# AbrahamSanders/realtime-codec-agent

Measured on AMD Instinct MI355X. Metric: batch-encode audio-hours/hour (+ xRT and p50 frame-step latency of 1 duplex stream in `duplex`), higher is better.
Workload: dtype f32; 1 GPU; batch MagiCodec-style encode, 16 kHz stereo, 0.1 s chunks / 2.0 s context, 256 windows per step (BASELINE configs[1]); codebook=131072x16

## Files before the change

include/rca.h:

```cpp
#ifndef RCA_H
#define RCA_H

#include <stdint.h>

#ifdef __cplusplus
extern "C" {
#endif

#define RCA_OK 0
#define RCA_ERR_ARG -1
#define RCA_ERR_HIP -2
#define RCA_ERR_STATE -3
#define RCA_ERR_MISSING -4

#define RCA_MAX_STAGES 8

typedef struct rca_codec rca_codec_t;
typedef struct rca_lm rca_lm_t;

#define RCA_F32 0
#define RCA_BF16 1
#define RCA_Q8_0 2
#define RCA_F16 3
#define RCA_Q6_K 5
// ... 44 lines not shown
                                     int64_t chunk_begin, int64_t chunk_end, int64_t* codes_dev,
                                     int64_t codes_per_channel, void* stream);

int rca_codec_encode_rows_dev(rca_codec_t* h, const float* audio_dev, const int64_t* src_off_dev, int32_t B, int32_t T, int32_t n_keep,
                              int64_t* codes_dev, const int64_t* dst_off_dev, int64_t span, void* stream);

int rca_codec_encode_tail_dev(rca_codec_t* h, const float* pcm_dev, int32_t B, int32_t T, int32_t n_keep,
                              int64_t* codes_dev, void* stream);
int rca_codec_decode_tail_dev(rca_codec_t* h, const int64_t* codes_dev, int32_t B, int32_t F, int32_t n_samples,
                              float* pcm_dev, void* stream);
int rca_codec_encode_tail(rca_codec_t* h, const float* pcm_host, int32_t B, int32_t T, int32_t n_keep, int64_t* codes_host);
int rca_codec_decode_tail(rca_codec_t* h, const int64_t* codes_host, int32_t B, int32_t F, int32_t n_samples, float* pcm_host);
int rca_codec_set_stream_graphs(rca_codec_t* h, int32_t enable);
int rca_codec_set_mfma_mode(rca_codec_t* h, int32_t mode);
int rca_codec_receptive_field(const rca_codec_t* h, int32_t* enc_left_frames, int32_t* dec_left_frames);
int rca_codec_set_window_trim(rca_codec_t* h, int32_t enable);

int rca_codec_decode(rca_codec_t* h, const int64_t* codes_host, int32_t B, int32_t F, float* pcm_host);
int rca_codec_decode_dev(rca_codec_t* h, const int64_t* codes_dev, int32_t B, int32_t F, float* pcm_dev,
                         void* stream);

int rca_codec_encoder_dev(rca_codec_t* h, const float* pcm_dev, int32_t B, int32_t T, float* ze_dev, void* stream);
int rca_codec_quantize_dev(rca_codec_t* h, const float* ze_dev, int64_t rows, int64_t* codes_dev, void* stream);
int rca_codec_decoder_dev(rca_codec_t* h, const float* zq_dev, int32_t B, int32_t F, float* pcm_dev, void* stream);
int rca_codec_codebook_dev(rca_codec_t* h, const float** out_dev);

int rca_codec_codebook(rca_codec_t* h, float* out_host);

int rca_codec_encode_tap(rca_codec_t* h, const float* pcm_host, int32_t B, int32_t T, int32_t layer,
                         float* out_host, int64_t out_numel);

int rca_codec_encode_tap_bf16(rca_codec_t* h, const float* pcm_host, int32_t B, int32_t T, int32_t layer,
                              uint16_t* hi_host, uint16_t* lo_host, int64_t numel);

int rca_codec_set_variant(rca_codec_t* h, int32_t variant);

int rca_codec_profile(rca_codec_t* h, int32_t enable);
int rca_codec_profile_read(rca_codec_t* h, int32_t kclass, double* total_ms, int64_t* launches, double* flops,
                           double* bytes);

typedef struct {
    int32_t vocab_size;
    int32_t hidden;
    int32_t n_layers;
    int32_t n_heads;
    int32_t n_kv_heads;
    int32_t head_dim;
    int32_t ffn;
    int32_t n_ctx;
    float rms_eps;
    float rope_theta;
    int32_t rope_scaling;
    float rope_factor;
    float rope_low_freq_factor;
    float rope_high_freq_factor;
    int32_t rope_orig_ctx;
    int32_t logits_all;
    int32_t decode_weights;
} rca_lm_config_t;

typedef struct {
    int32_t top_k;
    float top_p;
    float min_p;
    float temp;
    uint32_t seed;
// ... 78 lines not shown
```

realtime_codec_agent_amd/_native.py:

```python
from __future__ import annotations

import ctypes as C
import os
import subprocess
from typing import Dict, Iterable, List, Optional, Tuple

import numpy as np

_PKG_DIR = os.path.dirname(os.path.abspath(__file__))
CSRC_DIR = os.path.join(_PKG_DIR, "csrc")
LIB_PATH = os.environ.get("RCA_LIB_PATH") or os.path.join(_PKG_DIR, "librca_hip.so")
HIP_SOURCES = ["rca_codec.hip", "rca_lm.hip"]
HIPCC_FLAGS = ["--offload-arch=gfx950", "-O3", "-ffp-contract=off", "-std=c++17", "-fPIC", "-shared",
               "-Wno-unused-result", "-mllvm", "-amdgpu-kernarg-preload-count=14"]

MAX_STAGES = 8
RCA_F32, RCA_BF16, RCA_Q8_0, RCA_F16, RCA_Q4_K, RCA_Q6_K = 0, 1, 2, 3, 4, 5


class RcaError(RuntimeError):
    pass


class Q8Blocks:
# ... 215 lines not shown
                    print(" ".join(cmd))
                jobs.append((subprocess.Popen(cmd), cmd, obj))
        tmps = [obj + sfx for _, _, obj in jobs] + [LIB_PATH + sfx]
        try:
            failed = [cmd for p, cmd, _ in jobs if p.wait() != 0]
            if failed:
                raise subprocess.CalledProcessError(1, failed[0])
            for _, _, obj in jobs:
                os.replace(obj + sfx, obj)
            cmd = [hipcc, "--offload-arch=gfx950", "-shared", "-fPIC"] + objs + ["-o", LIB_PATH + sfx]
            if verbose:
                print(" ".join(cmd))
            subprocess.check_call(cmd)
            os.replace(LIB_PATH + sfx, LIB_PATH)
            with open(_stamp_path() + sfx, "w") as f:
                f.write(key + "\n")
            os.replace(_stamp_path() + sfx, _stamp_path())
        finally:
            for t in tmps + [_stamp_path() + sfx]:
                if os.path.exists(t):
                    os.remove(t)
    return LIB_PATH


_lib = None

ABI_SYMBOLS = [
    "rca_last_error", "rca_device_count", "rca_device_sync", "rca_version",
    "rca_codec_create", "rca_codec_destroy", "rca_codec_hop", "rca_codec_num_frames",
    "rca_codec_encode", "rca_codec_encode_dev", "rca_codec_encode_windows_dev", "rca_codec_encode_chunk_range_dev", "rca_codec_encode_rows_dev",
    "rca_codec_decode", "rca_codec_decode_dev",
    "rca_codec_encode_tail_dev", "rca_codec_decode_tail_dev", "rca_codec_encode_tail", "rca_codec_decode_tail", "rca_codec_set_stream_graphs", "rca_codec_receptive_field", "rca_codec_set_window_trim",
    "rca_codec_encoder_dev", "rca_codec_quantize_dev", "rca_codec_decoder_dev", "rca_codec_codebook_dev",
    "rca_codec_codebook", "rca_codec_encode_tap", "rca_codec_encode_tap_bf16", "rca_codec_set_variant", "rca_codec_sync",
    "rca_codec_profile", "rca_codec_profile_read",
    "rca_lm_create", "rca_lm_create_random", "rca_lm_destroy", "rca_lm_reset", "rca_lm_eval",
    "rca_lm_get_n_tokens", "rca_lm_set_n_tokens", "rca_lm_get_logits", "rca_lm_get_logits_row",
    "rca_lm_logits_dev", "rca_lm_sampler_init", "rca_lm_sample", "rca_lm_step", "rca_lm_token_probs",
    "rca_lm_sync", "rca_lm_set_graphs", "rca_lm_mask_head_rows", "rca_lm_set_mfma_prefill", "rca_lm_set_logits_all",
    "rca_lm_persist_codec_embeddings", "rca_lm_create_shared", "rca_lm_eval_async", "rca_lm_copy_kv", "rca_lm_swap_kv",
    "rca_lm_set_low_priority", "rca_lm_frame", "rca_lm_weight_format", "rca_lm_set_attn_fuse",
    "rca_duplex_frame", "rca_codec_workspace_sig", "rca_codec_stream_handoff", "rca_codec_codebook_size", "rca_codec_set_mfma_mode", "rca_lm_step_probe", "rca_duplex_prepare", "rca_duplex_precapture",
]


def lib():
    global _lib
    if _lib is not None:
        return _lib
    if not os.path.exists(LIB_PATH):
        raise RcaError(
            f"{LIB_PATH} not found: build the HIP extension first (python -c 'import __graft_entry__ as g; g.build()'). "
            "There is no CPU fallback for the product path."
        )
    import torch
    try:
        _lib = C.CDLL(LIB_PATH)
    except OSError as e:
        raise RcaError(f"cannot load {LIB_PATH}: {e}") from e
    _lib.rca_last_error.restype = C.c_char_p
    _lib.rca_version.restype = C.c_char_p
    return _lib


def check(rc: int, what: str = "") -> None:
    if rc != 0:
        msg = lib().rca_last_error()
# ... 40 lines not shown
```

realtime_codec_agent_amd/codec.py:

```python
from __future__ import annotations

import ctypes as C
from typing import Dict, Optional, Tuple

import numpy as np

from . import _native as N
from .codec_model import CodecConfig, init_codec_weights


class HipCodec:
    def __init__(self, cfg: CodecConfig, weights: Dict[str, np.ndarray], device: int = 0):
        self.cfg = cfg
        self.device = device
        self._lib = N.lib()
        self._h = C.c_void_p()
        tensors, keep = N.make_tensors(weights)
        ccfg = N.codec_config_c(cfg)
        N.check(self._lib.rca_codec_create(C.byref(ccfg), tensors, len(weights), device, C.byref(self._h)), "rca_codec_create")
        del keep
        self.hop = cfg.hop
        self.mfma_mode = 0

    def close(self):
# ... 59 lines not shown
    def set_mfma_mode(self, mode: int) -> None:
        N.check(self._lib.rca_codec_set_mfma_mode(self._h, int(mode)), "rca_codec_set_mfma_mode")
        self.mfma_mode = int(mode)

    def set_stream_graphs(self, enable: bool) -> None:
        N.check(self._lib.rca_codec_set_stream_graphs(self._h, int(bool(enable))), "rca_codec_set_stream_graphs")

    def codebook(self) -> np.ndarray:
        out = np.empty((self.cfg.codebook_size, self.cfg.codebook_dim), np.float32)
        N.check(self._lib.rca_codec_codebook(self._h, C.c_void_p(out.ctypes.data)), "rca_codec_codebook")
        return out

    def encode_tap(self, pcm: np.ndarray, layer: int) -> np.ndarray:
        pcm = np.ascontiguousarray(pcm, dtype=np.float32)
        B, T = pcm.shape
        F = self.num_frames(T)
        n = self.cfg.n_stages
        L = F * self.hop
        if layer == 0:
            shape = (B, self.cfg.channels[0], L)
        elif layer <= n:
            for i in range(layer):
                L //= self.cfg.strides[i]
            shape = (B, self.cfg.channels[layer], L)
        elif layer == n + 1:
            shape = (B, self.cfg.latent_dim, F)
        else:
            shape = (B * F, self.cfg.codebook_dim)
        out = np.empty(shape, np.float32)
        N.check(self._lib.rca_codec_encode_tap(self._h, C.c_void_p(pcm.ctypes.data), B, T, layer, C.c_void_p(out.ctypes.data),
                                               C.c_int64(out.size)), "rca_codec_encode_tap")
        return out

    def encode_tap_bf16(self, pcm: np.ndarray, layer: int) -> Tuple[np.ndarray, Optional[np.ndarray]]:
        pcm = np.ascontiguousarray(pcm, dtype=np.float32)
        B, T = pcm.shape
        L = self.num_frames(T) * self.hop
        for i in range(layer):
            L //= self.cfg.strides[i]
        Cn = self.cfg.channels[layer] if 0 <= layer <= self.cfg.n_stages else 0
        hi = np.empty((B, Cn // 16, L, 16), np.uint16)
        lo = np.empty_like(hi) if self.mfma_mode == 3 else None
        N.check(self._lib.rca_codec_encode_tap_bf16(self._h, C.c_void_p(pcm.ctypes.data), B, T, layer, C.c_void_p(hi.ctypes.data),
                                                    C.c_void_p(lo.ctypes.data if lo is not None else None), C.c_int64(B * Cn * L)),
                "rca_codec_encode_tap_bf16")
        unblock = lambda a: np.ascontiguousarray(a.transpose(0, 1, 3, 2).reshape(B, Cn, L))
        return unblock(hi), (unblock(lo) if lo is not None else None)

    def encode_dev(self, pcm_ptr: int, B: int, T: int, codes_ptr: int, stream: int = 0) -> None:
        N.check(self._lib.rca_codec_encode_dev(self._h, C.c_void_p(pcm_ptr), B, T, C.c_void_p(codes_ptr), C.c_void_p(stream)), "rca_codec_encode_dev")

    def decode_dev(self, codes_ptr: int, B: int, F: int, pcm_ptr: int, stream: int = 0) -> None:
        N.check(self._lib.rca_codec_decode_dev(self._h, C.c_void_p(codes_ptr), B, F, C.c_void_p(pcm_ptr), C.c_void_p(stream)), "rca_codec_decode_dev")

    def encode_tail_dev(self, pcm_ptr: int, B: int, T: int, n_keep: int, codes_ptr: int, stream: int = 0) -> None:
        N.check(self._lib.rca_codec_encode_tail_dev(self._h, C.c_void_p(pcm_ptr), B, T, n_keep, C.c_void_p(codes_ptr), C.c_void_p(stream)),
                "rca_codec_encode_tail_dev")

    def decode_tail_dev(self, codes_ptr: int, B: int, F: int, n_samples: int, pcm_ptr: int, stream: int = 0) -> None:
        N.check(self._lib.rca_codec_decode_tail_dev(self._h, C.c_void_p(codes_ptr), B, F, n_samples, C.c_void_p(pcm_ptr), C.c_void_p(stream)),
                "rca_codec_decode_tail_dev")

    def receptive_field(self) -> Tuple[int, int]:
        a, b = C.c_int32(), C.c_int32()
        N.check(self._lib.rca_codec_receptive_field(self._h, C.byref(a), C.byref(b)), "rca_codec_receptive_field")
        return a.value, b.value
# ... 199 lines not shown
```

realtime_codec_agent_amd/csrc/rca_codec.hip:

```cpp
#include <stdarg.h>

#include <algorithm>
#include <array>
#include <cmath>
#include <map>
#include <type_traits>

#include "rca_common.h"

namespace rca {
thread_local char g_err[512] = {0};
}
using namespace rca;

typedef float f32x16 __attribute__((ext_vector_type(16)));

#define RCA_LAT_MAX_FRAMES 64
#define RCA_LDS_BUDGET (152 * 1024)

typedef float f32x4 __attribute__((ext_vector_type(4)));

struct RowSrc {
    const float* base;
    int C;
// ... 683 lines not shown
                    char* const yr = reinterpret_cast<char*>(yw + (long)cu * orow);
                    *reinterpret_cast<float*>(yr + voff) = acc[wm][wn][r];
                }
        } else {
#pragma unroll
            for (int wm = 0; wm < WM; ++wm)
#pragma unroll
                for (int r = 0; r < 16; ++r) {
                    const int cu = wm * 32 + (r & 3) + 8 * (r >> 2);
                    char* const yr = reinterpret_cast<char*>(yw + (long)cu * orow);
                    if (co0 + cu + 4 * half < Cout) *reinterpret_cast<float*>(yr + voff) = acc[wm][wn][r];
                }
        }
    }
#ifdef RCA_CONV_TIMELINE
    if (tl_buf && lane == 0) {
        const long tl3 = (long)wall_clock64();
        const unsigned hw = __builtin_amdgcn_s_getreg((31 << 11) | (0 << 6) | 4);
        const unsigned xcc = __builtin_amdgcn_s_getreg((3 << 11) | (0 << 6) | 20);
        constexpr int region = KS == 4 ? 0 : KS == 8 ? 1 : KS == 10 ? 2 : KS == 16 ? 3 : KS == 3 ? 4 : 5;
        long* o = tl_buf + ((long)region * 65536 + ((blockIdx.x * RCA_CONV_WPB + wave) & 0xFFFF)) * 8;
        o[6] = tl_load | (tl_mfma << 32);
        o[7] = tl_write | ((long)nchunks << 32);
        o[0] = tl0; o[1] = tl1; o[2] = tl2; o[3] = tl3;
        o[4] = (long)hw | ((long)xcc << 32);
        o[5] = (long)KS | ((long)S << 8) | ((long)WM << 16) | ((long)wave << 24) | ((long)blockIdx.x << 32);
    }
#endif
}

template <int NWN, bool PRE>
__global__ __launch_bounds__(64, 2) void conv_first_mfma_kernel(const float* __restrict__ wp, const float* __restrict__ bias,
                                                               float* __restrict__ y, int Cout, int Lout, long Ncols, int post, float slope,
                                                               FuseIn fin) {
    constexpr int NW = NWN * 32;
    constexpr int E = (NW + 2) * 2;
    constexpr int NBLK = 2 * NWN + 1;
    constexpr int RS = 136;
    constexpr int ZERO = 128;
    constexpr int CIN = 32, KQ = CIN / 2;
    extern __shared__ __attribute__((aligned(16))) float ring[];
#ifdef RCA_CONV_TIMELINE
    long* const tl_buf = rca_prof_buf;
#endif
    RCA_TL_STAMP(tl0);
    const int lane = threadIdx.x & 63;
    const int half = lane >> 5, jl = lane & 31;
    const int n_co = Cout / 64;
    const long wg = blockIdx.x;
    const int xcd = (int)(wg & 7);
    const long seq = wg >> 3;
    const int co_tile = __builtin_amdgcn_readfirstlane((int)(seq % n_co));
    const long n0 = ((seq / n_co) * 8 + xcd) * NW;
    const int co0 = co_tile * 64;
    if (n0 >= Ncols) return;
    const long n_base = n0 > 0 ? n0 - 1 : 0;
    const int b_base = __builtin_amdgcn_readfirstlane((int)((unsigned)n_base / (unsigned)Lout));
    const int t_base = (int)(n_base - (long)b_base * Lout);
    const int lead = n0 > 0 ? 0 : 1;
    const long left = Ncols - n_base;
    const int ncol_left = left > NW + 2 ? NW + 2 : (int)left;
    auto rel_bt = [&](int dn, int& bb, int& tt) {
        int dt = dn + t_base;
        bb = dt >= Lout ? 1 : 0;
        tt = bb ? dt - Lout : dt;
    };

    const int ch_in = jl;
    float a_in[4];
#pragma unroll
    for (int m = 0; m < 4; ++m) a_in[m] = (2 * m + half < 7) ? fin.w_in[ch_in * 7 + 2 * m + half] : -0.0f;
    f32x16 b_in;
#pragma unroll
    for (int r = 0; r < 16; ++r) b_in[r] = fin.b_in[(r & 3) + 8 * (r >> 2) + 4 * half];
    long o0, o1;
    if (fin.src.row_off) {
        const long nrows = (Ncols + Lout - 1) / Lout;
        o0 = fin.src.row_off[b_base];
        o1 = fin.src.row_off[b_base + 1 < nrows ? b_base + 1 : b_base];
    } else {
        const int C = fin.src.C;
        const int c0 = b_base % C, w0 = b_base / C;
        const int c1 = c0 + 1 == C ? 0 : c0 + 1, w1 = c0 + 1 == C ? w0 + 1 : w0;
        o0 = (long)c0 * fin.src.chan_stride + (long)w0 * fin.src.win_stride;
        o1 = (long)c1 * fin.src.chan_stride + (long)w1 * fin.src.win_stride;
    }
    const long om = o0 < o1 ? o0 : o1;
    const rca_rsrc_t rs_pcm = rca_make_rsrc(fin.src.base + om, 0x7FFFFFFF);
    const unsigned prow0 = (unsigned)(o0 - om), prow1 = (unsigned)(o1 - om);
    constexpr unsigned OOB = 0x80000000u;
    auto pcm_load = [&](int bk, float (&pb)[4]) __attribute__((always_inline)) {
        const int e = 32 * bk + jl;
        const int dn = (e >> 1) - lead;
        const bool ok = e < E && dn >= 0 && dn < ncol_left;
        int bb, t;
        rel_bt(ok ? dn : 0, bb, t);
        const int i = 2 * t + (e & 1) - 3 + half;
        const unsigned ro = bb ? prow1 : prow0;
#pragma unroll
        for (int m = 0; m < 4; ++m) {
            const int j = i + 2 * m;
            const unsigned off = (ok && 2 * m + half < 7 && j >= 0 && j < fin.src.T) ? (ro + (unsigned)j) * 4u : OOB;
            pb[m] = rca_buffer_load_f32(rs_pcm, (int)off, 0, 0);
        }
    };
    auto cin_mfma = [&](int m, const float (&pb)[4], f32x16& d) __attribute__((always_inline)) {
        d = __builtin_amdgcn_mfma_f32_32x32x2f32(a_in[m], pb[m], m == 0 ? b_in : d, 0, 0, 0);
    };
    const int w_lane = 4 * half * RS + jl;
    auto cin_write = [&](int bk, f32x16& d, int r0, int r1) __attribute__((always_inline)) {
#pragma unroll
        for (int r = r0; r < r1; ++r) {
            float v = d[r];
            if (PRE) v = fmaxf(v, v * slope);
            ring[w_lane + ((r & 3) + 8 * (r >> 2)) * RS + ((32 * bk) & 127)] = v;
        }
    };

    if (lane < CIN) ring[lane * RS + ZERO] = 0.0f;
    float pa[4], pb[4];
    float4 a[2][KQ];
    {
        float p2[4];
        pcm_load(0, pa);
        pcm_load(1, pb);
        pcm_load(2, p2);
        __builtin_amdgcn_sched_barrier(0);
        const rca_rsrc_t rs_w = rca_make_rsrc(reinterpret_cast<const float4*>(wp) + (long)co_tile * 2 * KQ * 64, 0x7FFFFFFF);
#pragma unroll
        for (int wm = 0; wm < 2; ++wm)
#pragma unroll
            for (int q = 0; q < KQ; ++q) {
                const rca_f32x4_t v = rca_buffer_load_f32x4(rs_w, lane * 16, (wm * KQ + q) * 1024, 0);
                a[wm][q] = make_float4(v[0], v[1], v[2], v[3]);
            }
        __builtin_amdgcn_sched_barrier(0);
        f32x16 d0, d1;
#pragma unroll
        for (int m = 0; m < 4; ++m) { cin_mfma(m, pa, d0); cin_mfma(m, pb, d1); }
        cin_write(0, d0, 0, 16);
#pragma unroll
        for (int m = 0; m < 4; ++m) cin_mfma(m, p2, d0);
        cin_write(1, d1, 0, 16);
        cin_write(2, d0, 0, 16);
    }
    if (NBLK > 3) pcm_load(3, pa);
    if (NBLK > 4) pcm_load(4, pb);
    __builtin_amdgcn_wave_barrier();
    RCA_TL_STAMP(tl1);
#ifdef RCA_CONV_TIMELINE
    long tl_load = 1 << 30, tl_mfma = 0, tl_write = 0;
#endif

    const rca_rsrc_t rs_y = rca_make_rsrc(y + ((long)b_base * Cout + co0) * Lout, 0x7FFFFFFF);
    __builtin_amdgcn_s_setprio(RCA_CONV_EPRIO);
#pragma unroll
    for (int wn = 0; wn < NWN; ++wn) {
        RCA_TL_STAMP(ta);
        const int j = 32 * wn + jl;
        int bz, tz;
        rel_bt(1 - lead + j, bz, tz);
        const int ad0 = (half == 0 && tz == 0) ? ZERO : ((2 * j + 1 + half) & 127);
        const int ad1 = (half == 1 && tz == Lout - 1) ? ZERO : ((2 * j + 3 + half) & 127);
        f32x16 acc[2];
#pragma unroll
        for (int wm = 0; wm < 2; ++wm)
#pragma unroll
            for (int q = 0; q < 4; ++q) {
                const f32x4 bq = *reinterpret_cast<const f32x4*>(bias + co0 + wm * 32 + 8 * q + 4 * half);
#pragma unroll
                for (int jj = 0; jj < 4; ++jj) acc[wm][4 * q + jj] = bq[jj];
            }
        const bool more = 2 * wn + 4 < NBLK;
        f32x16 d;
        float bcur[4], bnxt[4];
        auto b_read = [&](int c, float (&bv)[4]) __attribute__((always_inline)) {
#pragma unroll
            for (int cl = 0; cl < 2; ++cl) {
                bv[2 * cl] = ring[ad0 + (2 * c + cl) * RS];
                bv[2 * cl + 1] = ring[ad1 + (2 * c + cl) * RS];
            }
        };
        b_read(0, bcur);
#pragma unroll
        for (int c = 0; c < KQ; ++c) {
            if (c + 1 < KQ) b_read(c + 1, bnxt);
#pragma unroll
            for (int kp = 0; kp < 4; ++kp) {
#pragma unroll
                for (int wm = 0; wm < 2; ++wm) {
                    const float4 q4 = a[wm][c];
                    const float av = kp == 0 ? q4.x : kp == 1 ? q4.y : kp == 2 ? q4.z : q4.w;
                    acc[wm] = __builtin_amdgcn_mfma_f32_32x32x2f32(av, bcur[kp], acc[wm], 0, 0, 0);
                }
                if (c == 0 && 2 * wn + 3 < NBLK) cin_mfma(kp, pa, d);
                if (c == 3 && more) cin_mfma(kp, pb, d);
            }
            if (c == 2 && 2 * wn + 3 < NBLK) cin_write(2 * wn + 3, d, 0, 16);
            if (more && c >= 4 && (c & 3) == 3) cin_write(2 * wn + 4, d, 4 * (c >> 2) - 4, 4 * (c >> 2));
            if (c == 1 && 2 * wn + 5 < NBLK) pcm_load(2 * wn + 5, pa);
            if (c == 4 && 2 * wn + 6 < NBLK) pcm_load(2 * wn + 6, pb);
            if (c + 1 < KQ) {
#pragma unroll
                for (int i = 0; i < 4; ++i) bcur[i] = bnxt[i];
            }
            __builtin_amdgcn_sched_barrier(0);
        }
        if (more) cin_write(2 * wn + 4, d, 12, 16);
        __builtin_amdgcn_wave_barrier();
        RCA_TL_STAMP(tb);
        const int dn = 1 - lead + j;
        int bb, t;
        rel_bt(dn, bb, t);
        const unsigned voff = dn < ncol_left ? ((unsigned)bb * (unsigned)(Cout * Lout) + (unsigned)t + (unsigned)(4 * half * Lout)) * 4u : OOB;
        if (post) {
#pragma unroll
            for (int wm = 0; wm < 2; ++wm)
#pragma unroll
                for (int r = 0; r < 16; ++r) acc[wm][r] = fmaxf(acc[wm][r], acc[wm][r] * slope);
        }
#pragma unroll
        for (int wm = 0; wm < 2; ++wm)
#pragma unroll
            for (int r = 0; r < 16; ++r) rca_buffer_store_f32(acc[wm][r], rs_y, (int)voff, (wm * 32 + (r & 3) + 8 * (r >> 2)) * Lout * 4, 0);
        RCA_TL_STAMP(tc);
        RCA_TL_MIN(tl_load, ta, tb); RCA_TL_ADD(tl_mfma, ta, tb); RCA_TL_ADD(tl_write, tb, tc);
    }
    if (RCA_CONV_EPRIO) __builtin_amdgcn_s_setprio(0);
    RCA_TL_STAMP(tl2);
#ifdef RCA_CONV_TIMELINE
    if (tl_buf && lane == 0) {
        const long tl3 = (long)wall_clock64();
        const unsigned hw = __builtin_amdgcn_s_getreg((31 << 11) | (0 << 6) | 4);
        const unsigned xcc = __builtin_amdgcn_s_getreg((3 << 11) | (0 << 6) | 20);
        long* o = tl_buf + ((long)blockIdx.x & 0xFFFF) * 8;
        o[6] = tl_load | (tl_mfma << 32);
        o[7] = tl_write | ((long)(2 * NWN) << 32);
        o[0] = tl0; o[1] = tl1; o[2] = tl2; o[3] = tl3;
        o[4] = (long)hw | ((long)xcc << 32);
        o[5] = 4L | (2L << 8) | (2L << 16) | ((long)blockIdx.x << 32);
    }
#endif
}

template <int KS, int S, int CIC, int FUSE>
__global__ __launch_bounds__(512) void conv1d_ws_kernel(const float* __restrict__ x, const float* __restrict__ wp,
                                                        const float* __restrict__ bias, float* __restrict__ y,
                                                        int Cin, int Lin, int Cout, int Lout, long Ncols, int nchunks,
                                                        int pre, float slope, FuseIn fin) {
    constexpr int WM = 2, WN = 2;
    constexpr int MT = WM * 32, NW = WN * 32;
    constexpr int U = ConvLds<S>::stride(NW);
    constexpr int KPC = CIC * KS / 2;
    constexpr int QPC = KPC / 4;
    constexpr int E = (NW + 2) * S;
    constexpr int RE = (E + 63) / 64;
    constexpr int padL = (KS - S + 1) / 2;
    constexpr int BUF = CIC * S * U + 4;
    constexpr int WBUF = WM * QPC * 64 * 4;
    static_assert(KPC % 4 == 0 && KPC <= 64, "chunk shape");

    extern __shared__ __attribute__((aligned(16))) float lds[];
    float* aw_all = lds;
    float* xs_all = lds + 2 * WBUF;

    const int lane = threadIdx.x & 63;
    const int half = lane >> 5;
    const int wave = __builtin_amdgcn_readfirstlane(threadIdx.x >> 6);
    const bool producer = wave >= 4;
    const int cw = wave & 3;
// ... 969 lines not shown
            for (int r = 0; r < 16; ++r) yr[(long)((r & 3) + 8 * (r >> 2)) * Lout] = acc[wm][wn][r];
        } else {
            const int Cbo = Cout / 16;
#pragma unroll
            for (int g = 0; g < 4; ++g) {
                float v[4];
#pragma unroll
                for (int j = 0; j < 4; ++j) {
                    const float a = acc[wm][wn][4 * g + j];
                    v[j] = act ? fmaxf(a, a * slope) : a;
                }
                const int ch = co0 + wm * 32 + 8 * g + 4 * half;
                const long o = (((long)b * Cbo + ch / 16) * Lout + t) * 16 + (ch & 15);
                const unsigned h0 = conv_pack_bf16x2(v[0], v[1]), h1 = conv_pack_bf16x2(v[2], v[3]);
                *reinterpret_cast<uint2*>(y_hi + o) = make_uint2(h0, h1);
                if (SPLIT) {
                    const unsigned l0 = conv_pack_bf16x2(v[0] - __uint_as_float(h0 << 16), v[1] - __uint_as_float(h0 & 0xffff0000u));
                    const unsigned l1 = conv_pack_bf16x2(v[2] - __uint_as_float(h1 << 16), v[3] - __uint_as_float(h1 & 0xffff0000u));
                    *reinterpret_cast<uint2*>(y_lo + o) = make_uint2(l0, l1);
                }
            }
        }
    }
}

struct Bf16Pack { conv_bf16raw* hi = nullptr; conv_bf16raw* lo = nullptr; float* w_in8 = nullptr; };

struct rca_codec {
    rca_codec_config_t cfg;
    int device = 0;
    hipStream_t stream = nullptr;
    int hop = 1;
    int variant = 1;
    int mfma_mode = 0;
    bool lat_mode = false;
    int enc_left_frames = 0, dec_left_frames = 0;
    bool window_trim = false;
    std::vector<ConvLayer> enc, dec;
    std::vector<Bf16Pack> bf16_packs;
    bool bf16_blk_split = true;
    float *q_in_w = nullptr, *q_in_b = nullptr;
    float *cb = nullptr, *hc = nullptr, *cbp = nullptr;
    DevBuf act[2], zbuf, keys, io_a, io_b, tail;
    void* pin = nullptr; size_t pin_cap = 0;
    struct StreamGraph { hipGraphExec_t exec = nullptr; int seen = 0; unsigned long long sig = 0; };
    std::map<std::array<int, 5>, StreamGraph> sgraphs;
    bool stream_graphs = true;
    int* err_flag = nullptr;
    hipStream_t last_stream = nullptr;
    bool last_stream_valid = false;
    hipEvent_t xev = nullptr;
    struct Prof { hipEvent_t a, b; int kclass; double flops, bytes; };
    bool profile = false;
    std::vector<Prof> prof;
    std::vector<Prof> prof_pool;
};

struct ProfScope {
    rca_codec* h; hipStream_t st; rca_codec::Prof p; bool on;
    ProfScope(rca_codec* h_, hipStream_t st_, int kclass, double flops, double bytes) : h(h_), st(st_), on(h_->profile) {
        if (!on) return;
        if (!h->prof_pool.empty()) { p = h->prof_pool.back(); h->prof_pool.pop_back(); }
        else { (void)hipEventCreate(&p.a); (void)hipEventCreate(&p.b); }
        p.kclass = kclass; p.flops = flops; p.bytes = bytes;
        (void)hipEventRecord(p.a, st);
    }
// ... 231 lines not shown
    if (hipMalloc((void**)&h->cb, (size_t)N * J * 4) != hipSuccess || hipMalloc((void**)&h->hc, (size_t)N * 4) != hipSuccess ||
        hipMalloc((void**)&h->cbp, (size_t)N * J * 4) != hipSuccess || hipMalloc((void**)&h->err_flag, 4) != hipSuccess) {
        free3();
        return bail(fail(RCA_ERR_HIP, "codebook alloc"));
    }
    (void)hipMemsetAsync(h->err_flag, 0, 4, h->stream);
#ifdef RCA_CONV_TIMELINE
    if (getenv("RCA_CONV_TIMELINE_OUT")) {
        long* b = nullptr;
        (void)hipMalloc((void**)&b, (size_t)(6 << 16) * 8 * 8);
        (void)hipMemset(b, 0, (size_t)(6 << 16) * 8 * 8);
        (void)hipMemcpyToSymbol(HIP_SYMBOL(rca_prof_buf), &b, 8);
    }
#endif
    codebook_proj_kernel<<<cdiv((long)N * J, 256), 256, 0, h->stream>>>(raw, pw, pb, h->cb, N, R, J);
    codebook_norm_pack_kernel<<<cdiv(N, 256), 256, 0, h->stream>>>(h->cb, h->hc, h->cbp, N, J);
    hipError_t e = hipStreamSynchronize(h->stream);
    free3();
    if (e != hipSuccess) return bail(fail(RCA_ERR_HIP, "codebook init: %s", hipGetErrorString(e)));
    *out = h;
    return RCA_OK;
}

extern "C" int rca_codec_hop(const rca_codec_t* h, int32_t* hop) {
    if (!h || !hop) return fail(RCA_ERR_ARG, "null");
    *hop = h->hop;
    return RCA_OK;
}
extern "C" int rca_codec_num_frames(const rca_codec_t* h, int32_t T, int32_t* F) {
    if (!h || !F || T < 0) return fail(RCA_ERR_ARG, "bad argument");
    *F = (T + h->hop - 1) / h->hop;
    return RCA_OK;
}
extern "C" int rca_codec_set_variant(rca_codec_t* h, int32_t v) {
    if (!h || v < 0 || v > 2) return fail(RCA_ERR_ARG, "variant must be 0, 1 or 2");
    h->variant = v;
    return RCA_OK;
}
extern "C" int rca_codec_sync(rca_codec_t* h) {
    if (!h) return fail(RCA_ERR_ARG, "null");
    RCA_HIP(hipSetDevice(h->device));
    RCA_HIP(hipStreamSynchronize(h->stream));
    return RCA_OK;
}

template <int KS, int S, int CIC, int WM, int WN, int FUSE, int TR, int BF = 0>
static void launch_conv_cfg(const ConvLayer& L, const float* wp, int nchunks, const float* x, float* y, int Lin, int Lc, long Ncols,
                            float slope, const FuseIn& fin, const TrInfo& tr, hipStream_t st, int act) {
    constexpr int NT = RCA_CONV_WPB * WN * 32, MT = WM * 32;
    constexpr int lds = RCA_CONV_WPB * 2 * (CIC * S * ConvLds<S>::stride(WN * 32) + 4) * 4;
    static_assert(lds <= 65536, "LDS budget");
    const long col_tiles = (cdiv(Ncols, NT) + 7) / 8 * 8;
    dim3 grid((unsigned)(col_tiles * cdiv(L.cout, MT) * (TR ? tr.s : 1)));
    if constexpr (!FUSE && !TR && BF == 0) {
        if (L.cin % CIC == 0 && nchunks * CIC == L.cin) {
            conv1d_mfma_kernel<KS, S, CIC, WM, WN, 0, 0, 0, 1><<<grid, 64 * RCA_CONV_WPB, lds, st>>>(x, wp, L.bp, y, L.cin, Lin, L.cout, Lc, Ncols, nchunks, act, slope, fin, tr);
            return;
        }
    }
    conv1d_mfma_kernel<KS, S, CIC, WM, WN, FUSE, TR, BF><<<grid, 64 * RCA_CONV_WPB, lds, st>>>(x, wp, L.bp, y, L.cin, Lin, L.cout, Lc, Ncols, nchunks, act, slope, fin, tr);
}

template <int KS, int S, int CIC>
static int launch_conv_mfma(const ConvLayer& L, const float* x, float* y, int B, int Lin, int Lout, float slope, hipStream_t st,
                            const FuseIn* fuse = nullptr, int act = -1, int bf = 0) {
    if (act < 0) act = L.pre;
    const long Ncols = (long)B * Lout;
    if (bf) {
        const FuseIn none_b{};
        const TrInfo notr_b{};
        const bool big = (long)cdiv(Ncols, 64) * cdiv(L.cout, 64) >= 2048;
#define RCA_BF_LAUNCH(FU, BFM) do { \
            if (big) launch_conv_cfg<KS, S, CIC, 2, 2, FU, 0, BFM>(L, L.wp, L.nchunks, x, y, Lin, Lout, Ncols, slope, FU ? *fuse : none_b, notr_b, st, act); \
            else launch_conv_cfg<KS, S, CIC, 1, 1, FU, 0, BFM>(L, L.wp, L.nchunks, x, y, Lin, Lout, Ncols, slope, FU ? *fuse : none_b, notr_b, st, act); } while (0)
        if constexpr (KS == 4 || KS == 8 || KS == 16) {
            if (fuse) { if (bf == 3) RCA_BF_LAUNCH(1, 3); else RCA_BF_LAUNCH(1, 1); RCA_LAUNCH_CHECK(); return RCA_OK; }
        }
        if (fuse) return fail(RCA_ERR_ARG, "internal: fused first layer of this shape has no bf16 instantiation");
        if (bf == 3) RCA_BF_LAUNCH(0, 3); else RCA_BF_LAUNCH(0, 1);
#undef RCA_BF_LAUNCH
        RCA_LAUNCH_CHECK();
        return RCA_OK;
    }
    const long waves_big = (long)cdiv(Ncols, 64) * cdiv(L.cout, 64);
#ifdef RCA_CONV_FORCE_MID
    constexpr long BIG_MIN = 1L << 40, MID_MIN = 2048;
#else
    constexpr long BIG_MIN = 8192, MID_MIN = 2048;
#endif
    const FuseIn none{};
    const TrInfo notr{};
    if (fuse) {
        static const bool wide = []() { const char* e = getenv("RCA_FUSE_WIDE"); return !(e && e[0] == '0'); }();
        if constexpr (KS == 4 && S == 2) {
            const char* mi = getenv("RCA_FUSE_MFMA_IN");
            constexpr int NWN = 4;
            if (!(mi && mi[0] == '0') && wide && waves_big >= BIG_MIN && Lout >= NWN * 32 + 3 && L.cin == 32 && L.cout % 64 == 0) {
                const long col_tiles = (cdiv(Ncols, NWN * 32) + 7) / 8 * 8;
                const dim3 grid((unsigned)(col_tiles * (L.cout / 64)));
                constexpr int lds = 32 * 136 * 4;
                if (act & 1) conv_first_mfma_kernel<NWN, true><<<grid, 64, lds, st>>>(L.wp, L.bp, y, L.cout, Lout, Ncols, act & 2, slope, *fuse);
                else conv_first_mfma_kernel<NWN, false><<<grid, 64, lds, st>>>(L.wp, L.bp, y, L.cout, Lout, Ncols, act & 2, slope, *fuse);
                RCA_LAUNCH_CHECK();
                return RCA_OK;
            }
            if (wide && waves_big >= BIG_MIN && Lout >= 131 && L.cin % 2 == 0) {
                launch_conv_cfg<4, 2, 2, 2, 4, 1, 0>(L, L.wp, L.cin / 2, x, y, Lin, Lout, Ncols, slope, *fuse, notr, st, act);
                RCA_LAUNCH_CHECK();
                return RCA_OK;
            }
        }
        if (waves_big >= BIG_MIN) launch_conv_cfg<KS, S, CIC, 2, 2, 1, 0>(L, L.wp, L.nchunks, x, y, Lin, Lout, Ncols, slope, *fuse, notr, st, act);
        else launch_conv_cfg<KS, S, CIC, 1, 1, 1, 0>(L, L.wp, L.nchunks, x, y, Lin, Lout, Ncols, slope, *fuse, notr, st, act);
    } else {
        if (waves_big >= BIG_MIN) launch_conv_cfg<KS, S, CIC, 2, 2, 0, 0>(L, L.wp, L.nchunks, x, y, Lin, Lout, Ncols, slope, none, notr, st, act);
        else if (waves_big >= MID_MIN) launch_conv_cfg<KS, S, CIC, 1, 2, 0, 0>(L, L.wp, L.nchunks, x, y, Lin, Lout, Ncols, slope, none, notr, st, act);
        else if (KS == 3 && L.cout >= 64 && waves_big >= 1024) launch_conv_cfg<KS, S, CIC, (KS == 3 ? 2 : 1), 1, 0, 0>(L, L.wp, L.nchunks, x, y, Lin, Lout, Ncols, slope, none, notr, st, act);
        else launch_conv_cfg<KS, S, CIC, 1, 1, 0, 0>(L, L.wp, L.nchunks, x, y, Lin, Lout, Ncols, slope, none, notr, st, act);
    }
    RCA_LAUNCH_CHECK();
    return RCA_OK;
}

static int launch_convtr_mfma(const ConvLayer& L, const float* x, float* y, int B, int Lin, float slope, hipStream_t st) {
    const int Lc = Lin + 1;
    const long Ncols = (long)B * Lc;
    const FuseIn none{};
    const TrInfo tr{L.s, (L.k - L.s + 1) / 2, Lin * L.s, L.cout_pad / 32};
    const long waves_big = (long)cdiv(Ncols, 64) * cdiv(L.cout, 64) * L.s;
    if (L.cout > 32 && waves_big >= 2048) launch_conv_cfg<2, 1, 16, 2, 2, 0, 1>(L, L.wp_tr, L.nchunks_tr, x, y, Lin, Lc, Ncols, slope, none, tr, st, L.pre);
    else launch_conv_cfg<2, 1, 16, 1, 1, 0, 1>(L, L.wp_tr, L.nchunks_tr, x, y, Lin, Lc, Ncols, slope, none, tr, st, L.pre);
    RCA_LAUNCH_CHECK();
    return RCA_OK;
}

template <int KS, int S, int CIC, int FUSE>
// ... 276 lines not shown
        max_elems = std::max(max_elems, (size_t)B * c.latent_dim * L);
    }
    int rc;
    if ((rc = h->act[0].ensure(max_elems * 4)) != RCA_OK) return rc;
    if ((rc = h->act[1].ensure(max_elems * 4)) != RCA_OK) return rc;
    if (bf16_blk_ok(h, tap_layer) && (double)B * max_elems < 4.0e18 && Tp / h->enc[1].s >= 64) {
        *F_out = F;
        return run_encoder_bf16(h, src, B, Tp, max_elems, st, ze_out, tap_layer, tap_dev, bf16_tap, bf16_planes);
    }
    if (bf16_tap >= 0) return fail(RCA_ERR_ARG, "bf16 tap: encode() does not take the blocked bf16 pipeline here (mfma mode %d, B=%d T=%d)", h->mfma_mode, B, src.T);
    int cur = 0;
    int L = Tp;
    size_t first = 1;
    const ConvLayer& E0 = h->enc[0];
    const ConvLayer& E1 = h->enc[1];
    const bool fuse01 = !h->lat_mode && h->variant >= 1 && tap_layer != 0 && E0.k == 7 && E1.wp && E1.k == 2 * E1.s && (double)B * E1.cin * L < 4.0e9 &&
                        ((E1.k == 4 && E1.s == 2) || (E1.k == 8 && E1.s == 4) || (E1.k == 16 && E1.s == 8)) && L / E1.s >= 67 &&
                        (double)E1.cout * (L / E1.s) < 2.6e8 &&
                        (src.row_off ? (double)src.span : (double)src.C * (double)std::labs(src.chan_stride) + (double)std::labs(src.win_stride) + src.T) < 5.0e8;
    bool prev_post = false;
    auto handoff = [&](size_t next, int Lnext) {
        return tap_layer < 0 && h->variant == 1 && !h->lat_mode && next < h->enc.size() && h->enc[next].pre && mfma_conv_ok(h, h->enc[next], B, Lnext, 0);
    };
    if (fuse01) {
        float* y = h->act[cur].as<float>();
        FuseIn fin{src, E0.w, E0.b};
        const float slope = c.leaky_slope;
        const int Lout = L / E1.s;
        {
            ProfScope ps(h, st, 0, 2.0 * E1.cin * E1.k * E1.cout * (double)B * Lout + 2.0 * E0.k * E0.cout * (double)B * L,
                         4.0 * ((double)B * src.T + (double)B * E1.cout * Lout + (double)E1.cin * E1.k * E1.cout));
            prev_post = handoff(2, Lout);
            const int act = (E1.pre ? 1 : 0) | (prev_post ? 2 : 0);
            if (h->variant == 2 && try_conv_ws(E1, nullptr, y, B, L, Lout, slope, st, &fin)) { rc = RCA_OK; RCA_LAUNCH_CHECK(); }
            else if (E1.k == 4) rc = launch_conv_mfma<4, 2, 4>(E1, nullptr, y, B, L, Lout, slope, st, &fin, act, h->mfma_mode);
            else if (E1.k == 8) rc = launch_conv_mfma<8, 4, RCA_CIC_K8>(E1, nullptr, y, B, L, Lout, slope, st, &fin, act, h->mfma_mode);
            else rc = launch_conv_mfma<16, 8, RCA_CIC_K16>(E1, nullptr, y, B, L, Lout, slope, st, &fin, act, h->mfma_mode);
        }
        if (rc != RCA_OK) return rc;
        L = Lout;
        first = 2;
        if (tap_layer == 1) RCA_HIP(hipMemcpyAsync(tap_dev, y, (size_t)B * E1.cout * L * 4, hipMemcpyDeviceToDevice, st));
    } else if (h->lat_mode && !src.row_off && src.win_stride == 0 && src.C == B &&
               try_conv_lds(h, h->enc[0], src.base, src.chan_stride, src.T, h->act[cur].as<float>(), B, L, 0, st)) {
        RCA_LAUNCH_CHECK();
    } else {
        const ConvLayer& L0 = h->enc[0];
        const long total = (long)B * L;
        float* y = h->act[cur].as<float>();
        ProfScope ps(h, st, 2, 2.0 * L0.k * L0.cout * (double)total, 4.0 * ((double)total + (double)total * L0.cout));
        if (L0.k == 7) conv_in_kernel<7><<<cdiv(total, 256), 256, 0, st>>>(src, L0.w, L0.b, y, B, L0.cout, L);
        else if (L0.k == 5) conv_in_kernel<5><<<cdiv(total, 256), 256, 0, st>>>(src, L0.w, L0.b, y, B, L0.cout, L);
        else conv_in_kernel<3><<<cdiv(total, 256), 256, 0, st>>>(src, L0.w, L0.b, y, B, L0.cout, L);
        RCA_LAUNCH_CHECK();
        if (tap_layer == 0) RCA_HIP(hipMemcpyAsync(tap_dev, y, (size_t)B * L0.cout * L * 4, hipMemcpyDeviceToDevice, st));
    }
    for (size_t li = first; li < h->enc.size(); ++li) {
        const ConvLayer& Ly = h->enc[li];
        float* x = h->act[cur].as<float>();
        float* y = h->act[cur ^ 1].as<float>();
        bool done = false;
        if ((rc = run_conv(h, Ly, x, y, B, L, 0, st, prev_post, handoff(li + 1, L / Ly.s), &done)) != RCA_OK) return rc;
        prev_post = done;
        L /= Ly.s;
        cur ^= 1;
        if (tap_layer == (int)li) RCA_HIP(hipMemcpyAsync(tap_dev, y, (size_t)B * Ly.cout * L * 4, hipMemcpyDeviceToDevice, st));
    }
    *ze_out = h->act[cur].as<float>();
// ... 534 lines not shown
```

Measured before the change: 3284 audio-hours/hour.

## Let fused first-conv MFMA kernel stream a runtime number of column groups

The fused conv0+conv1 MFMA kernel now accepts a runtime group count (NWN=0 path), so each workgroup covers 8 or 16 column groups of 32 instead of a fixed 4. This amortizes per-block prologue work (ring setup, first PCM loads, bias loads) over more output columns, and bias is staged in LDS for the dynamic path. The group loop is restructured into first/middle/last calls with compile-time pipelining flags. The costs are fewer workgroups, possibly less latency hiding, and a non-unrolled inner loop. A query API exposing the chosen group count is also added.

```diff
diff --git a/include/rca.h b/include/rca.h
--- a/include/rca.h
+++ b/include/rca.h
@@ -100,6 +100,8 @@
 
 int rca_codec_encode_tap_bf16(rca_codec_t* h, const float* pcm_host, int32_t B, int32_t T, int32_t layer,
                               uint16_t* hi_host, uint16_t* lo_host, int64_t numel);
+
+int rca_codec_last_fuse_groups(rca_codec_t* h, int32_t* groups);
 
 int rca_codec_set_variant(rca_codec_t* h, int32_t variant);
 
diff --git a/realtime_codec_agent_amd/_native.py b/realtime_codec_agent_amd/_native.py
--- a/realtime_codec_agent_amd/_native.py
+++ b/realtime_codec_agent_amd/_native.py
@@ -271,7 +271,7 @@
     "rca_codec_decode", "rca_codec_decode_dev",
     "rca_codec_encode_tail_dev", "rca_codec_decode_tail_dev", "rca_codec_encode_tail", "rca_codec_decode_tail", "rca_codec_set_stream_graphs", "rca_codec_receptive_field", "rca_codec_set_window_trim",
     "rca_codec_encoder_dev", "rca_codec_quantize_dev", "rca_codec_decoder_dev", "rca_codec_codebook_dev",
-    "rca_codec_codebook", "rca_codec_encode_tap", "rca_codec_encode_tap_bf16", "rca_codec_set_variant", "rca_codec_sync",
+    "rca_codec_codebook", "rca_codec_encode_tap", "rca_codec_encode_tap_bf16", "rca_codec_last_fuse_groups", "rca_codec_set_variant", "rca_codec_sync",
     "rca_codec_profile", "rca_codec_profile_read",
     "rca_lm_create", "rca_lm_create_random", "rca_lm_destroy", "rca_lm_reset", "rca_lm_eval",
     "rca_lm_get_n_tokens", "rca_lm_set_n_tokens", "rca_lm_get_logits", "rca_lm_get_logits_row",
diff --git a/realtime_codec_agent_amd/codec.py b/realtime_codec_agent_amd/codec.py
--- a/realtime_codec_agent_amd/codec.py
+++ b/realtime_codec_agent_amd/codec.py
@@ -115,6 +115,11 @@
                                                C.c_int64(out.size)), "rca_codec_encode_tap")
         return out
 
+    def last_fuse_groups(self) -> int:
+        g = C.c_int32(-1)
+        N.check(self._lib.rca_codec_last_fuse_groups(self._h, C.byref(g)), "rca_codec_last_fuse_groups")
+        return int(g.value)
+
     def encode_tap_bf16(self, pcm: np.ndarray, layer: int) -> Tuple[np.ndarray, Optional[np.ndarray]]:
         pcm = np.ascontiguousarray(pcm, dtype=np.float32)
         B, T = pcm.shape
diff --git a/realtime_codec_agent_amd/csrc/rca_codec.hip b/realtime_codec_agent_amd/csrc/rca_codec.hip
--- a/realtime_codec_agent_amd/csrc/rca_codec.hip
+++ b/realtime_codec_agent_amd/csrc/rca_codec.hip
@@ -739,13 +739,12 @@
 template <int NWN, bool PRE>
 __global__ __launch_bounds__(64, 2) void conv_first_mfma_kernel(const float* __restrict__ wp, const float* __restrict__ bias,
                                                                float* __restrict__ y, int Cout, int Lout, long Ncols, int post, float slope,
-                                                               FuseIn fin) {
-    constexpr int NW = NWN * 32;
-    constexpr int E = (NW + 2) * 2;
-    constexpr int NBLK = 2 * NWN + 1;
+                                                               int groups, FuseIn fin) {
+    const int GW = NWN ? NWN : groups;
     constexpr int RS = 136;
     constexpr int ZERO = 128;
     constexpr int CIN = 32, KQ = CIN / 2;
+    constexpr int BIAS = CIN * RS;
     extern __shared__ __attribute__((aligned(16))) float ring[];
 #ifdef RCA_CONV_TIMELINE
     long* const tl_buf = rca_prof_buf;
@@ -758,9 +757,12 @@
     const int xcd = (int)(wg & 7);
     const long seq = wg >> 3;
     const int co_tile = __builtin_amdgcn_readfirstlane((int)(seq % n_co));
-    const long n0 = ((seq / n_co) * 8 + xcd) * NW;
+    const long n0 = ((seq / n_co) * 8 + xcd) * (GW * 32);
     const int co0 = co_tile * 64;
     if (n0 >= Ncols) return;
+    const int G = NWN ? NWN : __builtin_amdgcn_readfirstlane(Ncols - n0 < (long)GW * 32 ? (int)((Ncols - n0 + 31) >> 5) : GW);
+    const int NW = G * 32;
+    const int E = (NW + 2) * 2;
     const long n_base = n0 > 0 ? n0 - 1 : 0;
     const int b_base = __builtin_amdgcn_readfirstlane((int)((unsigned)n_base / (unsigned)Lout));
     const int t_base = (int)(n_base - (long)b_base * Lout);
@@ -825,6 +827,7 @@
     };
 
     if (lane < CIN) ring[lane * RS + ZERO] = 0.0f;
+    if (NWN == 0) ring[BIAS + lane] = bias[co0 + lane];
     float pa[4], pb[4];
     float4 a[2][KQ];
     {
@@ -851,8 +854,11 @@
         cin_write(1, d1, 0, 16);
         cin_write(2, d0, 0, 16);
     }
-    if (NBLK > 3) pcm_load(3, pa);
-    if (NBLK > 4) pcm_load(4, pb);
+    if (NWN == 0) __builtin_amdgcn_s_waitcnt(0x0F70);
+    if (G > 1) {
+        pcm_load(3, pa);
+        pcm_load(4, pb);
+    }
     __builtin_amdgcn_wave_barrier();
     RCA_TL_STAMP(tl1);
 #ifdef RCA_CONV_TIMELINE
@@ -861,8 +867,8 @@
 
     const rca_rsrc_t rs_y = rca_make_rsrc(y + ((long)b_base * Cout + co0) * Lout, 0x7FFFFFFF);
     __builtin_amdgcn_s_setprio(RCA_CONV_EPRIO);
-#pragma unroll
-    for (int wn = 0; wn < NWN; ++wn) {
+    auto group = [&](const int wn, auto next_c, auto load_c) __attribute__((always_inline)) {
+        constexpr bool NEXT = decltype(next_c)::value, LOAD = decltype(load_c)::value;
         RCA_TL_STAMP(ta);
         const int j = 32 * wn + jl;
         int bz, tz;
@@ -874,11 +880,11 @@
         for (int wm = 0; wm < 2; ++wm)
 #pragma unroll
             for (int q = 0; q < 4; ++q) {
-                const f32x4 bq = *reinterpret_cast<const f32x4*>(bias + co0 + wm * 32 + 8 * q + 4 * half);
+                const f32x4 bq = NWN == 0 ? *reinterpret_cast<const f32x4*>(ring + BIAS + wm * 32 + 8 * q + 4 * half)
+                                          : *reinterpret_cast<const f32x4*>(bias + co0 + wm * 32 + 8 * q + 4 * half);
 #pragma unroll
                 for (int jj = 0; jj < 4; ++jj) acc[wm][4 * q + jj] = bq[jj];
             }
-        const bool more = 2 * wn + 4 < NBLK;
         f32x16 d;
         float bcur[4], bnxt[4];
         auto b_read = [&](int c, float (&bv)[4]) __attribute__((always_inline)) {
@@ -900,20 +906,20 @@
                     const float av = kp == 0 ? q4.x : kp == 1 ? q4.y : kp == 2 ? q4.z : q4.w;
                     acc[wm] = __builtin_amdgcn_mfma_f32_32x32x2f32(av, bcur[kp], acc[wm], 0, 0, 0);
                 }
-                if (c == 0 && 2 * wn + 3 < NBLK) cin_mfma(kp, pa, d);
-                if (c == 3 && more) cin_mfma(kp, pb, d);
-            }
-            if (c == 2 && 2 * wn + 3 < NBLK) cin_write(2 * wn + 3, d, 0, 16);
-            if (more && c >= 4 && (c & 3) == 3) cin_write(2 * wn + 4, d, 4 * (c >> 2) - 4, 4 * (c >> 2));
-            if (c == 1 && 2 * wn + 5 < NBLK) pcm_load(2 * wn + 5, pa);
-            if (c == 4 && 2 * wn + 6 < NBLK) pcm_load(2 * wn + 6, pb);
+                if (c == 0 && NEXT) cin_mfma(kp, pa, d);
+                if (c == 3 && NEXT) cin_mfma(kp, pb, d);
+            }
+            if (c == 2 && NEXT) cin_write(2 * wn + 3, d, 0, 16);
+            if (NEXT && c >= 4 && (c & 3) == 3) cin_write(2 * wn + 4, d, 4 * (c >> 2) - 4, 4 * (c >> 2));
+            if (c == 1 && LOAD) pcm_load(2 * wn + 5, pa);
+            if (c == 4 && LOAD) pcm_load(2 * wn + 6, pb);
             if (c + 1 < KQ) {
 #pragma unroll
                 for (int i = 0; i < 4; ++i) bcur[i] = bnxt[i];
             }
             __builtin_amdgcn_sched_barrier(0);
         }
-        if (more) cin_write(2 * wn + 4, d, 12, 16);
+        if (NEXT) cin_write(2 * wn + 4, d, 12, 16);
         __builtin_amdgcn_wave_barrier();
         RCA_TL_STAMP(tb);
         const int dn = 1 - lead + j;
@@ -932,7 +938,18 @@
             for (int r = 0; r < 16; ++r) rca_buffer_store_f32(acc[wm][r], rs_y, (int)voff, (wm * 32 + (r & 3) + 8 * (r >> 2)) * Lout * 4, 0);
         RCA_TL_STAMP(tc);
         RCA_TL_MIN(tl_load, ta, tb); RCA_TL_ADD(tl_mfma, ta, tb); RCA_TL_ADD(tl_write, tb, tc);
-    }
+    };
+    constexpr std::true_type yes{};
+    constexpr std::false_type no{};
+    if (G > 2) {
+        group(0, yes, yes);
+#pragma unroll(NWN ? NWN : 1)
+        for (int wn = 1; wn < G - 2; ++wn) group(wn, yes, yes);
+        group(G - 2, yes, no);
+    } else if (G == 2) {
+        group(0, yes, no);
+    }
+    group(G - 1, no, no);
     if (RCA_CONV_EPRIO) __builtin_amdgcn_s_setprio(0);
     RCA_TL_STAMP(tl2);
 #ifdef RCA_CONV_TIMELINE
@@ -942,7 +959,7 @@
         const unsigned xcc = __builtin_amdgcn_s_getreg((3 << 11) | (0 << 6) | 20);
         long* o = tl_buf + ((long)blockIdx.x & 0xFFFF) * 8;
         o[6] = tl_load | (tl_mfma << 32);
-        o[7] = tl_write | ((long)(2 * NWN) << 32);
+        o[7] = tl_write | ((long)(2 * G) << 32);
         o[0] = tl0; o[1] = tl1; o[2] = tl2; o[3] = tl3;
         o[4] = (long)hw | ((long)xcc << 32);
         o[5] = 4L | (2L << 8) | (2L << 16) | ((long)blockIdx.x << 32);
@@ -1978,6 +1995,7 @@
     hipStream_t stream = nullptr;
     int hop = 1;
     int variant = 1;
+    int last_fuse_groups = 0;
     int mfma_mode = 0;
     bool lat_mode = false;
     int enc_left_frames = 0, dec_left_frames = 0;
@@ -2275,6 +2293,12 @@
     *F = (T + h->hop - 1) / h->hop;
     return RCA_OK;
 }
+extern "C" int rca_codec_last_fuse_groups(rca_codec_t* h, int32_t* groups) {
+    if (!h || !groups) return fail(RCA_ERR_ARG, "null argument");
+    *groups = h->last_fuse_groups;
+    return RCA_OK;
+}
+
 extern "C" int rca_codec_set_variant(rca_codec_t* h, int32_t v) {
     if (!h || v < 0 || v > 2) return fail(RCA_ERR_ARG, "variant must be 0, 1 or 2");
     h->variant = v;
@@ -2306,7 +2330,7 @@
 
 template <int KS, int S, int CIC>
 static int launch_conv_mfma(const ConvLayer& L, const float* x, float* y, int B, int Lin, int Lout, float slope, hipStream_t st,
-                            const FuseIn* fuse = nullptr, int act = -1, int bf = 0) {
+                            const FuseIn* fuse = nullptr, int act = -1, int bf = 0, int* fuse_groups = nullptr) {
     if (act < 0) act = L.pre;
     const long Ncols = (long)B * Lout;
     if (bf) {
@@ -2339,12 +2363,37 @@
             const char* mi = getenv("RCA_FUSE_MFMA_IN");
             constexpr int NWN = 4;
             if (!(mi && mi[0] == '0') && wide && waves_big >= BIG_MIN && Lout >= NWN * 32 + 3 && L.cin == 32 && L.cout % 64 == 0) {
-                const long col_tiles = (cdiv(Ncols, NWN * 32) + 7) / 8 * 8;
+                const char* fs = getenv("RCA_FUSE_STREAM");
+                int G = NWN;
+                if (!(fs && fs[0] == '0')) {
+                    for (int g = 16; g >= 8; g >>= 1)
+                        if (Lout >= g * 32 + 3 && cdiv(Ncols, g * 32) * (L.cout / 64) >= 2048) { G = g; break; }
+                }
+#ifdef RCA_FUSE_SWEEP
+                bool unroll8 = false;
+                if (const char* e = getenv("RCA_FUSE_SWEEP_G")) {
+                    const int g = atoi(e);
+                    if ((g == 4 || g == 8 || g == 16 || g == 32) && Lout >= g * 32 + 3) G = g;
+                    unroll8 = G == 8 && e[1] == 'u';
+                }
+#endif
+                const long col_tiles = (cdiv(Ncols, G * 32) + 7) / 8 * 8;
                 const dim3 grid((unsigned)(col_tiles * (L.cout / 64)));
-                constexpr int lds = 32 * 136 * 4;
-                if (act & 1) conv_first_mfma_kernel<NWN, true><<<grid, 64, lds, st>>>(L.wp, L.bp, y, L.cout, Lout, Ncols, act & 2, slope, *fuse);
-                else conv_first_mfma_kernel<NWN, false><<<grid, 64, lds, st>>>(L.wp, L.bp, y, L.cout, Lout, Ncols, act & 2, slope, *fuse);
+                constexpr int lds = (32 * 136 + 64) * 4;
+                if (G == NWN) {
+                    if (act & 1) conv_first_mfma_kernel<NWN, true><<<grid, 64, lds, st>>>(L.wp, L.bp, y, L.cout, Lout, Ncols, act & 2, slope, NWN, *fuse);
+                    else conv_first_mfma_kernel<NWN, false><<<grid, 64, lds, st>>>(L.wp, L.bp, y, L.cout, Lout, Ncols, act & 2, slope, NWN, *fuse);
+#ifdef RCA_FUSE_SWEEP
+                } else if (unroll8) {
+                    if (act & 1) conv_first_mfma_kernel<8, true><<<grid, 64, lds, st>>>(L.wp, L.bp, y, L.cout, Lout, Ncols, act & 2, slope, 8, *fuse);
+                    else conv_first_mfma_kernel<8, false><<<grid, 64, lds, st>>>(L.wp, L.bp, y, L.cout, Lout, Ncols, act & 2, slope, 8, *fuse);
+#endif
+                } else {
+                    if (act & 1) conv_first_mfma_kernel<0, true><<<grid, 64, lds, st>>>(L.wp, L.bp, y, L.cout, Lout, Ncols, act & 2, slope, G, *fuse);
+                    else conv_first_mfma_kernel<0, false><<<grid, 64, lds, st>>>(L.wp, L.bp, y, L.cout, Lout, Ncols, act & 2, slope, G, *fuse);
+                }
                 RCA_LAUNCH_CHECK();
+                if (fuse_groups) *fuse_groups = G;
                 return RCA_OK;
             }
             if (wide && waves_big >= BIG_MIN && Lout >= 131 && L.cin % 2 == 0) {
@@ -2687,8 +2736,9 @@
                          4.0 * ((double)B * src.T + (double)B * E1.cout * Lout + (double)E1.cin * E1.k * E1.cout));
             prev_post = handoff(2, Lout);
             const int act = (E1.pre ? 1 : 0) | (prev_post ? 2 : 0);
+            h->last_fuse_groups = 0;
             if (h->variant == 2 && try_conv_ws(E1, nullptr, y, B, L, Lout, slope, st, &fin)) { rc = RCA_OK; RCA_LAUNCH_CHECK(); }
-            else if (E1.k == 4) rc = launch_conv_mfma<4, 2, 4>(E1, nullptr, y, B, L, Lout, slope, st, &fin, act, h->mfma_mode);
+            else if (E1.k == 4) rc = launch_conv_mfma<4, 2, 4>(E1, nullptr, y, B, L, Lout, slope, st, &fin, act, h->mfma_mode, &h->last_fuse_groups);
             else if (E1.k == 8) rc = launch_conv_mfma<8, 4, RCA_CIC_K8>(E1, nullptr, y, B, L, Lout, slope, st, &fin, act, h->mfma_mode);
             else rc = launch_conv_mfma<16, 8, RCA_CIC_K16>(E1, nullptr, y, B, L, Lout, slope, st, &fin, act, h->mfma_mode);
         }
```

Result: no change. 3308 audio-hours/hour, median of 6 (+0.7%).
